# dselivanov/rsparse

Hardware: AMD Instinct MI355X
Metric: als_iterations_per_sec (higher is better)
Workload: dtype f32 (Gram products of rows > 512 / <= 32 non-zeros as 2 x fp16 / 3 x bf16 split terms of the fp32 operands, fp32 accumulate; everything else fp32); 1 GPU; WRMF implicit ALS, CG(3), synthetic 10000000x1000000, 500155883 nnz, rank 128, lambda 0.1; survey_config=3, feedback=implicit, n_items=1000000, nnz=500155883, rank=128, solver=conjugate_gradient, cg_steps=3, parallelism=rows sharded x1, factors replicated

## Files before the change

rsparse_amd/csrc/wrmf_cgp.hip:

```cpp
#include "wrmf_internal.h"
#include "wrmf_device.h"

namespace rsparse_hip {
namespace {

using namespace dev;

constexpr int kPairMaxSweeps = 4;

template <int NQ, bool QUAD = false>
struct PairSmem {
  static constexpr int KP = 128, ps = KP + 8, os = QUAD ? KP + 8 : KP + 4;
  static constexpr int cols = QUAD ? 16 : 8;
  static constexpr int pcs = QUAD ? 2 * ps : ps;
  static constexpr size_t gfrag = NQ == 16 ? (size_t)4 * 16 * 1024 : 0;
  static constexpr size_t nxt = NQ == 16 ? (size_t)4 * 2 * 2 * 64 * 4 : 0;
  static constexpr size_t pub = (size_t)2 * cols * ps * 2, out = (size_t)cols * os * 4;
  static_assert(!QUAD || (pub == out && (size_t)pcs * 2 == (size_t)os * 4), "QUAD: one column, one stretch of LDS");
  static constexpr size_t bytes = gfrag + (QUAD ? pub : pub + out) + (size_t)4 * 8 * NQ * 4 + nxt + 16;
};
static_assert(PairSmem<16>::bytes <= 81920 && PairSmem<16, true>::bytes <= 81920, "two workgroups per CU");

template <bool GB, bool KFULL = false, int NQ = 8, bool QUAD = false>
__global__ __launch_bounds__(256, 2) void als_cgp_kernel(AlsArgs a, const int32_t* __restrict__ rows, int n_rows, int iters,
// ... 294 lines not shown
            } else {
              ah = *reinterpret_cast<const f16x8*>(sGf + ((t * 4 + ks) * 2 + 0) * 1024 + (QUAD ? ln : lane) * 16);
              al = *reinterpret_cast<const f16x8*>(sGf + ((t * 4 + ks) * 2 + 1) * 1024 + (QUAD ? ln : lane) * 16);
            }
            d0[t] = __builtin_amdgcn_mfma_f32_16x16x32_f16(ah, bh, d0[t], 0, 0, 0);
            d1[t] = __builtin_amdgcn_mfma_f32_16x16x32_f16(ah, bl, d1[t], 0, 0, 0);
            d1[t] = __builtin_amdgcn_mfma_f32_16x16x32_f16(al, bh, d1[t], 0, 0, 0);
          }
        }
        if (QUAD || (lane & 15) < 8) {
#pragma unroll
          for (int t = 0; t < 2; t++) {
            const f32x4 d = (d0[t] + d1[t]) * ginv;
            float* po = QUAD ? sOut + li * SM::os + 32 * wv + 16 * t + 4 * lg : sOut + (lane & 15) * SM::os + 32 * wv + 16 * t + 4 * (lane >> 4);
            *reinterpret_cast<f32x4*>(po) = d;
          }
        }
      }
      float lacc = 0.f;
      if (mode != 2) {
        float* trec = (mode == 0 ? tacc : tcur) + gs;
#pragma unroll
        for (int q0 = 0; q0 < NQ; q0 += 4) {
          if (blk_on(q0)) {
            float t[4];
            f32x2 s2[4];
#pragma unroll
            for (int u = 0; u < 4; u++) s2[u] = f32x2{0.f, 0.f};
#pragma unroll
            for (int rr = 0; rr < RPN; rr += 2) {
              const f32x2 va = {v[rr], v[rr + 1]};
#pragma unroll
              for (int u = 0; u < 4; u++) {
                const f32x2 xa = {xt[q0 + u][rr], xt[q0 + u][rr + 1]};
                s2[u] = __builtin_elementwise_fma(xa, va, s2[u]);
              }
            }
#pragma unroll
            for (int u = 0; u < 4; u++) t[u] = s2[u].x + s2[u].y;
#pragma unroll
            for (int u = 0; u < 4; u++) t[u] += dpp<0xB1>(t[u]);
#pragma unroll
            for (int u = 0; u < 4; u++) t[u] += dpp<0x4E>(t[u]);
#pragma unroll
            for (int u = 0; u < 4; u++) t[u] += dpp<0x141>(t[u]);
#pragma unroll
            for (int u = 0; u < 4; u++) t[u] += dpp<0x140>(t[u]);
#pragma unroll
            for (int u = 0; u < 4; u++) {
              const int q = q0 + u;
              const float c = GREG ? cv[q] : (QUAD ? nx[64 + q] : nx[64 + 2 * q + g2]);
              trec[SS * q] = t[u];
              const float w = mode == 0 ? c - (c - 1.f) * (GB ? t[u] + gbias : t[u]) : (c - 1.f) * t[u];
#pragma unroll
              for (int rr = 0; rr < RPN; rr++) acc[rr] = fmaf(w, xt[q][rr], acc[rr]);
            }
          }
        }
      } else {
        wave_sync();
        const float t = tacc[lslot];
        const float dd = ltgt - t;
        const float ls = row16_sum((lgrp && lslot < cnt) ? cl * dd * dd : 0.f);
        lacc = QUAD ? ls : pair_sum(ls);
      }
      if (mode != 2) {
        __syncthreads();
        const float f = (QUAD || g2 == 0) ? vinv : 0.f;
#pragma unroll
        for (int b = 0; b < NV; b++) {
          const float* po = QUAD ? sOut + lcol * SM::os + b * 16 * VW + li * VW : sOut + col * SM::os + b * 16 * VW + i * VW;
          const f32x4 o = *reinterpret_cast<const f32x4*>(po);
#pragma unroll
          for (int c = 0; c < VW; c++) acc[b * VW + c] = fmaf(f, o[c], acc[b * VW + c]);
        }
#pragma unroll
        for (int rr = 0; rr < RPN; rr++) out[rr] = QUAD ? acc[rr] : pair_sum(acc[rr]);
        if constexpr (GB) {
          if (mode == 0) {
#pragma unroll
            for (int b = 0; b < NV; b++) {
              const int off = b * 16 * VW + i * VW;
              const float4 pc = *reinterpret_cast<const float4*>(a.rhs_init + min(off, k - VW));
              const float* pf = reinterpret_cast<const float*>(&pc);
#pragma unroll
              for (int c = 0; c < VW; c++) out[b * VW + c] += off < k ? pf[c] : 0.f;
            }
          }
        }
      } else {
        loss_out = lacc;
      }
    };
    auto dot16 = [&](const float(&u)[RPN], const float(&w)[RPN]) {
      float s = 0.f;
#pragma unroll
      for (int rr = 0; rr < RPN; rr++) s = fmaf(u[rr], w[rr], s);
      return row16_sum(s);
    };

    float dummy = 0.f;
    sweep(x, 0, r, dummy);
    if constexpr (KFULL)
      request_indices(it + 1 < iters && ridx(it + 1) < n_rows, p1_c, p2_c - p1_c, (it + 1) & 1);
#pragma unroll
    for (int rr = 0; rr < RPN; rr++) p[rr] = r[rr];
    float rsold = dot16(r, r);
    bool conv = !live;
    for (int itc = 0; itc < a.cg_steps; ++itc) {
      sweep(p, 1, ap, dummy);
      const float pap = dot16(p, ap);
      const float alpha = conv ? 0.f : (float)((double)rsold / (double)pap);
      wave_sync();
      if (lgrp) tacc[lslot] = fmaf(alpha, tcur[lslot], tacc[lslot]);
      wave_sync();
#pragma unroll
      for (int rr = 0; rr < RPN; rr++) {
        x[rr] = fmaf(alpha, p[rr], x[rr]);
        r[rr] = fmaf(-alpha, ap[rr], r[rr]);
      }
      const float rsnew = dot16(r, r);
      if (!conv) {
        if (rsnew < kCgTol) {
          conv = true;
        } else {
          const float beta = (float)((double)rsnew / (double)rsold);
#pragma unroll
          for (int rr = 0; rr < RPN; rr++) p[rr] = fmaf(p[rr], beta, r[rr]);
          rsold = rsnew;
        }
      }
    }
    float rl = 0.f;
    sweep(x, 2, ap, rl);
    if constexpr (KFULL) {
      settle_indices();
    }
    if (live) {
      const float xx = dot16(x, x);
      wloss += (double)rl + a.lambda_loss * (double)xx;
      if (QUAD || g2 == 0) {
#pragma unroll
        for (int b = 0; b < NV; b++) {
          const int off = b * 16 * VW + i * VW;
          if (off < k) {
            float4 pc;
            float* pf = reinterpret_cast<float*>(&pc);
#pragma unroll
            for (int c = 0; c < VW; c++) pf[c] = x[b * VW + c];
            *reinterpret_cast<float4*>(yrow + off) = pc;
          }
        }
      }
    }
  }
  const double other = __shfl(wloss, 32);
  if constexpr (QUAD) {
    const double wsum = (wloss + __shfl(wloss, 16)) + (other + __shfl(wloss, 48));
    if (lane == 0) a.loss_partials[loss_slot0 + (size_t)blockIdx.x * 4 + wv] = wsum;
  } else {
    if (lane == 0) a.loss_partials[loss_slot0 + (size_t)blockIdx.x * 4 + wv] = wloss + other;
  }
}

}

bool cgp_supported(int k, bool implicit) { return implicit && k > 64 && k <= 128 && k % 4 == 0; }
bool cgp_wide_supported(int k, bool implicit, bool gbias) { return implicit && k == 128 && !gbias; }
bool cgp_quad_supported(int k, bool implicit, bool gbias) { return implicit && k == 128 && !gbias; }

hipError_t launch_als_cgp(const AlsArgs& a, const int32_t* rows, int n_rows, CgpForm form, size_t loss_slot0, hipStream_t s,
                          hipEvent_t* ev_slot) {
  const int rpw = cgp_rows_per_wave(form);
  const int grid = cgp_grid(n_rows, rpw);
  if (grid <= 0) return hipSuccess;
  const int iters = cgp_visits(n_rows, rpw);
  const bool gb = a.gbias != 0.f;
  const bool full = !gb && a.k == 128;
  const bool wide = form == kCgpWide, quad = form == kCgpQuad;
  if ((wide || quad) && !full) return hipErrorInvalidValue;
  auto k0 = als_cgp_kernel<false, false>;
  auto k0f = als_cgp_kernel<false, true>;
  auto k1 = als_cgp_kernel<true, false>;
  auto kw = als_cgp_kernel<false, true, 16>;
  auto kq = als_cgp_kernel<false, true, 16, true>;
  const void* fn = quad ? reinterpret_cast<const void*>(kq) : wide ? reinterpret_cast<const void*>(kw)
                        : gb ? reinterpret_cast<const void*>(k1) : (full ? reinterpret_cast<const void*>(k0f) : reinterpret_cast<const void*>(k0));
  const size_t lds = quad ? PairSmem<16, true>::bytes : wide ? PairSmem<16>::bytes : PairSmem<8>::bytes;
  hipError_t err = hipFuncSetAttribute(fn, hipFuncAttributeMaxDynamicSharedMemorySize, (int)lds);
  if (err != hipSuccess) return err;
  prof_note(ev_slot, fn);
  if (quad) hipLaunchKernelGGL(kq, dim3(grid), dim3(256), lds, s, a, rows, n_rows, iters, loss_slot0);
  else if (wide) hipLaunchKernelGGL(kw, dim3(grid), dim3(256), lds, s, a, rows, n_rows, iters, loss_slot0);
  else if (gb) hipLaunchKernelGGL(k1, dim3(grid), dim3(256), lds, s, a, rows, n_rows, iters, loss_slot0);
  else if (full) hipLaunchKernelGGL(k0f, dim3(grid), dim3(256), lds, s, a, rows, n_rows, iters, loss_slot0);
  else hipLaunchKernelGGL(k0, dim3(grid), dim3(256), lds, s, a, rows, n_rows, iters, loss_slot0);
  return hipGetLastError();
}

}
```

rsparse_amd/csrc/wrmf_cgq.hip:

```cpp
#include <algorithm>

#include "wrmf_internal.h"
#include "wrmf_device.h"

namespace rsparse_hip {
namespace {

using namespace dev;

constexpr int kGvFirstMinCapq = 16;
constexpr int kStreamPrefixQ = 4;
constexpr int kIdxPrefetchMaxWpr = 2;

constexpr int kMaxSavedSweeps = 4;

template <int KP>
struct QG {
  static constexpr int RPN = KP / 16;
  static constexpr int VW = RPN >= 4 ? 4 : RPN;
  static constexpr int NV = RPN / VW;
  __device__ static __forceinline__ int elem(int i, int r) { return (r / VW) * (16 * VW) + i * VW + (r % VW); }
};

template <int VW>
struct Piece;
template <>
struct Piece<4> { using type = float4; };
template <>
struct Piece<2> { using type = float2; };

__device__ __forceinline__ float groups_reduce_scatter4(const float a0, const float a1, const float a2, const float a3) {
  const auto s01 = __builtin_amdgcn_permlane16_swap(__float_as_uint(a0), __float_as_uint(a1), false, false);
  const float c = __uint_as_float(s01[0]) + __uint_as_float(s01[1]);
  const auto s23 = __builtin_amdgcn_permlane16_swap(__float_as_uint(a2), __float_as_uint(a3), false, false);
  const float d = __uint_as_float(s23[0]) + __uint_as_float(s23[1]);
  const auto t = __builtin_amdgcn_permlane32_swap(__float_as_uint(c), __float_as_uint(d), false, false);
  return __uint_as_float(t[0]) + __uint_as_float(t[1]);
}
template <int KP, int CAPQ, int WAVES, int WPR, int STREAM, bool IMPLICIT, int DMF = 0>
struct QSmem {
  static constexpr size_t gram_floats = (IMPLICIT && DMF != 1) ? (size_t)KP * KP : 0;
  static constexpr size_t vec_floats = IMPLICIT ? (size_t)WAVES * KP : 0;
  static constexpr size_t red_floats = WPR > 1 ? (size_t)2 * WAVES * KP + 2 * WAVES : 0;
  static constexpr bool cv_lds = !STREAM && CAPQ * (KP / 16) > 128;
  static constexpr bool wideq = !STREAM && CAPQ * (KP / 16) > 160;
  static constexpr size_t tsv_floats = (STREAM && !IMPLICIT) ? 0 : (size_t)WAVES * (cv_lds ? 3 : 2) * CAPQ * 4;
  static constexpr size_t pre_floats = STREAM ? (size_t)WAVES * kStreamPrefixQ * 4 * KP : 0;
  static constexpr int dmf_ps = KP + 8, dmf_os = KP + 4;
  static constexpr size_t dmf_floats = DMF ? (size_t)WAVES * dmf_ps + (size_t)WAVES * dmf_os : 0;
  static constexpr size_t pfx_floats =
      (!STREAM && WPR > kIdxPrefetchMaxWpr && (CAPQ == 16 || CAPQ == 20 || CAPQ == 24)) ? (size_t)WAVES * 2 * CAPQ * 4 : 0;
  static constexpr size_t wl_floats = cv_lds ? (size_t)WAVES * 2 : 0;
  static constexpr size_t xs_floats = cv_lds ? (size_t)WAVES * KP : 0;
  static constexpr size_t bytes =
      (gram_floats + vec_floats + red_floats + tsv_floats + pre_floats + dmf_floats + pfx_floats + wl_floats + xs_floats) * 4 + 16;
};

template <int KP, int CAPQ, int WAVES, int WPR, int STREAM, bool IMPLICIT, int DMF = 0, bool GB = false, bool KFULL = false>
__global__ __launch_bounds__(WAVES * 64, 2) void als_cgq_kernel(AlsArgs a, const int32_t* __restrict__ rows, int n_rows,
                                                             int rows_per_team, size_t loss_slot0) {
  using G_ = QG<KP>;
  constexpr int RPN = G_::RPN, VW = G_::VW, NV = G_::NV, CAP = CAPQ * 4, TEAMS = WAVES / WPR;
  using piece_t = typename Piece<VW>::type;
  using SM = QSmem<KP, CAPQ, WAVES, WPR, STREAM, IMPLICIT, DMF>;
  static_assert(WAVES % WPR == 0, "teams must tile the workgroup");
  constexpr bool GRS = RPN == 8 && VW == 4;
  auto groups_all_reduce8 = [](float(&a8)[RPN]) {
    if constexpr (RPN == 8) {
      const float r0 = groups_reduce_scatter4(a8[0], a8[1], a8[2], a8[3]);
      const float r1 = groups_reduce_scatter4(a8[4], a8[5], a8[6], a8[7]);
      float g0[4], g1[4];
      rows_to_all<4>(r0, g0);
      rows_to_all<4>(r1, g1);
#pragma unroll
      for (int e = 0; e < 4; e++) a8[e] = g0[e], a8[4 + e] = g1[e];
    }
  };
  static_assert(!DMF || (IMPLICIT && KP == 128 && WAVES == 4 && WPR == 1 && STREAM == 0), "DMF geometry");
  static_assert(DMF != 1 || CAPQ == 8, "register-resident G terms: only the 8-quad kernel has the 64 registers");
  static_assert(!GB || IMPLICIT, "the global bias of explicit feedback is removed from the data (R/model_WRMF.R:278-282)");
  const float gbias = GB ? a.gbias : 0.f, ltgt = GB ? a.loss_tgt_const : 1.f;
  extern __shared__ __attribute__((aligned(16))) char smem[];
  float* sG = reinterpret_cast<float*>(smem);
  float* sVec = sG + SM::gram_floats;
  float* sRed = sVec + SM::vec_floats;
  float* sRedL = sRed + (WPR > 1 ? 2 * WAVES * KP : 0);
  float* sTsv = sVec + SM::vec_floats + SM::red_floats;
  float* sPre = sTsv + SM::tsv_floats;
  float* sPfx = sPre + SM::pre_floats;
  _Float16* sPh = reinterpret_cast<_Float16*>(sPre + SM::pre_floats);
  _Float16* sPl = sPh + WAVES * SM::dmf_ps;
  float* sOut = reinterpret_cast<float*>(sPl + WAVES * SM::dmf_ps);

  const int tid = threadIdx.x, lane = tid & 63, wv = rfl(tid >> 6);
  const int g = lane >> 4, i = lane & 15;
  const int team = wv / WPR, tw = wv % WPR;
  const int k = KFULL ? KP : a.k;
  if constexpr (IMPLICIT && DMF == 0) {
    constexpr int GU = (KP * KP) % (8 * WAVES * 64) == 0 ? 8 : ((KP * KP) % (2 * WAVES * 64) == 0 ? 2 : 1);
    static_assert((KP * KP) % (GU * WAVES * 64) == 0, "the Gramian copy walks whole batches");
    for (int e0 = tid; e0 < KP * KP; e0 += GU * WAVES * 64) {
      float gv[GU];
#pragma unroll
      for (int u = 0; u < GU; u++) {
        const int e = e0 + u * WAVES * 64, r = e / KP, c = e % KP;
        gv[u] = a.XtX[(size_t)min(r, k - 1) * k + min(c, k - 1)];
      }
#pragma unroll
      for (int u = 0; u < GU; u++) {
// ... 138 lines not shown
    float cl[CVLDS ? 1 : NSL];
#pragma unroll
    for (int s2 = 0; s2 < (CVLDS ? 1 : NSL); s2++) cl[s2] = 0.f;
    auto csv_fill = [&](auto&& conf_of, const int n) {
      const int ln = opaque_lane<WIDEQ>(lane);
#pragma unroll
      for (int s2 = 0; s2 < NSL; s2++) {
        const int sl = ln + 64 * s2;
        if (s2 == 0 || sl < CAP) csv[(sl & 3) * CAPQ + (sl >> 2)] = sl < n ? conf_of(sl) : 0.f;
      }
    };
    int ccnt = 0;

    constexpr bool ZPAD = STREAM == 0;
    constexpr bool TSAVE = STREAM == 0;
    constexpr bool GVFIRST = STREAM == 0 && CAPQ >= kGvFirstMinCapq;
    constexpr bool IDXPF = CAP <= 64 && ((STREAM == 0 && WPR <= kIdxPrefetchMaxWpr) || (STREAM == 1 && IMPLICIT));
    constexpr bool DMAPF = KFULL && !IDXPF && SM::pfx_floats > 0;
    int* pfxI = reinterpret_cast<int*>(sPfx) + wv * 2 * CAP;
    float* pfxC = sPfx + wv * 2 * CAP + CAP;
    auto dma_slot = [&](const int j0, const int n) {
      const int j = j0 + min(lane, n - 1);
      dma4(a.row_idx + j, lds_addr(pfxI));
      dma4(a.vals + j, lds_addr(pfxC));
      if constexpr (CAP > 64) {
        if (lane < CAP - 64) {
          const int j2 = j0 + min(lane + 64, n - 1);
          dma4(a.row_idx + j2, lds_addr(pfxI + 64));
          dma4(a.vals + j2, lds_addr(pfxC + 64));
        }
      }
    };
    int pf_pos = -1;
#define RSP_SLOT_IN(q, n) (SM::wideq ? g < (n) - 4 * (q) : 4 * (q) + g < (n))
#define RSP_SLOT_J(q, n) max(SM::wideq ? min(g, (n) - 1 - 4 * (q)) + 4 * (q) : min(4 * (q) + g, (n) - 1), 0)
    auto gather_q = [&](auto nq_tag, const int base, const int n, const bool from_pf = false) {
      constexpr int NQG = decltype(nq_tag)::value;
      int id[NQG > 0 ? NQG : 1];
      if constexpr (DMAPF) {
        if (!from_pf && n > 0) {
          dma_slot(base, n);
          wait_vm<0>();
        }
        wave_sync();
#pragma unroll
        for (int q = 0; q < NQG; q++) {
          const int j = RSP_SLOT_J(q, n);
          id[q] = pfxI[j];
          if constexpr (!CVLDS) cv[q] = (!ZPAD || RSP_SLOT_IN(q, n)) ? pfxC[j] : 0.f;
        }
        if constexpr (CVLDS) {
          csv_fill([&](int sl) { return pfxC[sl]; }, n);
        } else if constexpr (TSAVE) {
#pragma unroll
          for (int s2 = 0; s2 < NSL; s2++) cl[s2] = lane + 64 * s2 < n ? pfxC[min(lane + 64 * s2, CAP - 1)] : 0.f;
        }
        wave_sync();
      } else if (IDXPF && from_pf) {
        int* xi = reinterpret_cast<int*>(tacc);
        wave_sync();
        xi[lane & (CAP - 1)] = pf_id;
        tcur[lane & (CAP - 1)] = pf_c;
        wave_sync();
#pragma unroll
        for (int q = 0; q < NQG; q++) {
          const int j = RSP_SLOT_J(q, n);
          id[q] = xi[j];
          if constexpr (!CVLDS) cv[q] = (!ZPAD || RSP_SLOT_IN(q, n)) ? tcur[j] : 0.f;
        }
        if constexpr (TSAVE) cl[0] = lane < n ? pf_c : 0.f;
        wave_sync();
      } else {
#pragma unroll
        for (int q = 0; q < NQG; q++) {
          const int j = RSP_SLOT_J(q, n);
          id[q] = a.row_idx[base + j];
          if constexpr (!CVLDS) {
            const float c = a.vals[base + j];
            cv[q] = (!ZPAD || RSP_SLOT_IN(q, n)) ? c : 0.f;
          }
        }
        if constexpr (CVLDS) {
          wave_sync();
          csv_fill([&](int sl) { return a.vals[base + sl]; }, n);
          wave_sync();
        } else if constexpr (TSAVE) {
#pragma unroll
          for (int s2 = 0; s2 < NSL; s2++) cl[s2] = lane + 64 * s2 < n ? a.vals[base + lane + 64 * s2] : 0.f;
        }
      }
      const int ig = (SM::wideq && !KFULL) ? (opaque_lane<true>(lane) & 15) : i;
#pragma unroll
      for (int q = 0; q < NQG; q++) {
        const float* src = (!ZPAD || RSP_SLOT_IN(q, n)) ? a.X + (size_t)id[q] * k : a.zero_row;
#pragma unroll
        for (int b = 0; b < NV; b++) {
          const int off = b * 16 * VW + ig * VW;
          if constexpr (KFULL) {
            const piece_t pc = *reinterpret_cast<const piece_t*>(src + off);
            const float* pf = reinterpret_cast<const float*>(&pc);
#pragma unroll
            for (int c = 0; c < VW; c++) xt[q][b * VW + c] = pf[c];
          } else {
            const piece_t pc = *reinterpret_cast<const piece_t*>(src + min(off, k - VW));
            const float* pf = reinterpret_cast<const float*>(&pc);
#pragma unroll
            for (int c = 0; c < VW; c++) xt[q][b * VW + c] = off < k ? pf[c] : 0.f;
          }
// ... 66 lines not shown

    if constexpr (!WS_FIRST) load_warm_start();

    auto quad_pass = [&](const float(&v)[RPN], const int mode, float(&acc)[RPN], float& lacc, float* tsave) {
      float* trec = (mode == 0 ? tacc : tcur) + g;
      constexpr int QB = 4;
#pragma unroll
      for (int q0 = 0; q0 < CAPQ; q0 += QB) {
        if (4 * q0 < ccnt) {
          float t[QB];
          f32x2 s2[QB];
#pragma unroll
          for (int u = 0; u < QB; u++) s2[u] = f32x2{0.f, 0.f};
#pragma unroll
          for (int rr = 0; rr < RPN; rr += 2) {
            const f32x2 va = {v[rr], v[rr + 1]};
#pragma unroll
            for (int u = 0; u < QB; u++) {
              const f32x2 xa = {xt[q0 + u][rr], xt[q0 + u][rr + 1]};
              s2[u] = __builtin_elementwise_fma(xa, va, s2[u]);
            }
          }
#pragma unroll
          for (int u = 0; u < QB; u++) t[u] = s2[u].x + s2[u].y;
#pragma unroll
          for (int u = 0; u < QB; u++) t[u] += dpp<0xB1>(t[u]);
#pragma unroll
          for (int u = 0; u < QB; u++) t[u] += dpp<0x4E>(t[u]);
#pragma unroll
          for (int u = 0; u < QB; u++) t[u] += dpp<0x141>(t[u]);
#pragma unroll
          for (int u = 0; u < QB; u++) t[u] += dpp<0x140>(t[u]);
          float cq[QB];
          if constexpr (CVLDS) {
            const float4 c4 = *reinterpret_cast<const float4*>(csv + g * CAPQ + q0);
            cq[0] = c4.x; cq[1] = c4.y; cq[2] = c4.z; cq[3] = c4.w;
          } else {
#pragma unroll
            for (int u = 0; u < QB; u++) cq[u] = cv[q0 + u];
          }
#pragma unroll
          for (int u = 0; u < QB; u++) {
            const int q = q0 + u;
            const bool valid = ZPAD || 4 * q + g < ccnt;
            const float c = cq[u];
            if constexpr (STREAM == 1) {
              if (tsave && valid && i == 0) tsave[4 * q + g] = t[u];
            } else if constexpr (TSAVE) {
              trec[4 * q] = t[u];
            }
            if (mode == 2) {
              const float d = IMPLICIT ? ltgt - t[u] : c - t[u];
              lacc += valid ? (IMPLICIT ? c * d * d : d * d) : 0.f;
            } else {
              float w;
              if (mode == 0) w = IMPLICIT ? c - (c - 1.f) * (GB ? t[u] + gbias : t[u]) : c - t[u];
              else w = IMPLICIT ? (c - 1.f) * t[u] : t[u];
              w = valid ? w : 0.f;
#pragma unroll
              for (int rr = 0; rr < RPN; rr++) acc[rr] = fmaf(w, xt[q][rr], acc[rr]);
            }
          }
        }
      }
    };

    auto sweep = [&](const float(&v)[RPN], const int mode, float(&out)[RPN], float& loss_out, const bool live,
                     const int sidx = 0) {
      float acc[RPN];
#pragma unroll
      for (int rr = 0; rr < RPN; rr++) acc[rr] = 0.f;
      float lacc = 0.f;
      float vinv = 0.f;
      if constexpr (DMF) {
        if (mode != 2) {
          float vmax = 0.f;
#pragma unroll
          for (int rr = 0; rr < RPN; rr++) vmax = fmaxf(vmax, fabsf(v[rr]));
          vmax = row16_max(vmax);
          const int ve = fp16_scale_exp(vmax);
          const float vs = __uint_as_float((unsigned)ve << 23);
          vinv = __uint_as_float((unsigned)(254 - ve) << 23) * (mode == 0 ? -1.f : 1.f);
          if (g < NV) {
            float w4[VW];
#pragma unroll
            for (int c = 0; c < VW; c++) w4[c] = (g == 0 ? v[c] : v[VW + c]) * vs;
            unsigned h0, l0, h1, l1;
            split_f16(w4[0], w4[1], h0, l0);
            split_f16(w4[2], w4[3], h1, l1);
            const int off = wv * SM::dmf_ps + g * 16 * VW + i * VW;
            *reinterpret_cast<uint2*>(sPh + off) = make_uint2(h0, h1);
            *reinterpret_cast<uint2*>(sPl + off) = make_uint2(l0, l1);
          }
          __syncthreads();
          f32x4 d0[2], d1[2];
#pragma unroll
          for (int t = 0; t < 2; t++) d0[t] = d1[t] = f32x4{0.f, 0.f, 0.f, 0.f};
          const int nb = (lane & 3) * SM::dmf_ps + 8 * (lane >> 4);
#pragma unroll
          for (int ks = 0; ks < 4; ks++) {
            const f16x8 bh = *reinterpret_cast<const f16x8*>(sPh + nb + 32 * ks);
            const f16x8 bl = *reinterpret_cast<const f16x8*>(sPl + nb + 32 * ks);
#pragma unroll
            for (int t = 0; t < 2; t++) {
              f16x8 ah, al;
              if constexpr (DMF == 1) {
                ah = gAh[t][ks];
                al = gAl[t][ks];
              } else {
                ah = *reinterpret_cast<const f16x8*>(sGf + ((t * 4 + ks) * 2 + 0) * 1024 + lane * 16);
                al = *reinterpret_cast<const f16x8*>(sGf + ((t * 4 + ks) * 2 + 1) * 1024 + lane * 16);
              }
              d0[t] = __builtin_amdgcn_mfma_f32_16x16x32_f16(ah, bh, d0[t], 0, 0, 0);
              d1[t] = __builtin_amdgcn_mfma_f32_16x16x32_f16(ah, bl, d1[t], 0, 0, 0);
              d1[t] = __builtin_amdgcn_mfma_f32_16x16x32_f16(al, bh, d1[t], 0, 0, 0);
            }
          }
          if ((lane & 15) < 4) {
#pragma unroll
            for (int t = 0; t < 2; t++) {
              const f32x4 d = (d0[t] + d1[t]) * ginv;
              *reinterpret_cast<f32x4*>(sOut + (lane & 15) * SM::dmf_os + 32 * wv + 16 * t + 4 * (lane >> 4)) = d;
            }
          }
        }
      }
      if (live) {
        if constexpr (IMPLICIT && !DMF) {
          if (mode != 2) {
            wave_sync();
            if (g == 0) {
#pragma unroll
              for (int b = 0; b < NV; b++) {
                piece_t pc;
                float* pf = reinterpret_cast<float*>(&pc);
#pragma unroll
                for (int c = 0; c < VW; c++) pf[c] = v[b * VW + c];
                *reinterpret_cast<piece_t*>(vec + b * 16 * VW + i * VW) = pc;
              }
            }
            wave_sync();
          }
        }
        auto dense_part = [&]() {
          if (IMPLICIT && !DMF && mode != 2) {
            const float sign = mode == 0 ? -1.f : 1.f;
            if constexpr (NRES > 0) {
#pragma unroll
              for (int rs = 0; rs < NRES; rs++) {
                const int kk = 4 * (g + 4 * rs);
                const float4 vb = *reinterpret_cast<const float4*>(vec + kk);
                const float vv[4] = {sign * vb.x, sign * vb.y, sign * vb.z, sign * vb.w};
#pragma unroll
                for (int u = 0; u < 4; u++)
#pragma unroll
                  for (int b = 0; b < NV; b++) {
                    const float* pf = reinterpret_cast<const float*>(&gres[rs][u][b]);
#pragma unroll
                    for (int c = 0; c < VW; c++) acc[b * VW + c] = fmaf(vv[u], pf[c], acc[b * VW + c]);
                  }
              }
            }
            for (int s4 = tw * 4 + g + 4 * NRES; s4 < KP / 4; s4 += WPR * 4) {
              const int kk = 4 * s4;
              const float4 vb = *reinterpret_cast<const float4*>(vec + kk);
              const float vv[4] = {sign * vb.x, sign * vb.y, sign * vb.z, sign * vb.w};
#pragma unroll
              for (int u = 0; u < 4; u++) {
                const float* grow = sG + (kk + u) * KP;
#pragma unroll
                for (int b = 0; b < NV; b++) {
                  const piece_t pc = *reinterpret_cast<const piece_t*>(grow + b * 16 * VW + i * VW);
                  const float* pf = reinterpret_cast<const float*>(&pc);
#pragma unroll
                  for (int c = 0; c < VW; c++) acc[b * VW + c] = fmaf(vv[u], pf[c], acc[b * VW + c]);
                }
              }
            }
          }
        };
        if constexpr (GVFIRST) dense_part();
        if (resident) {
          if (mode != 2 || !TSAVE) {
            quad_pass(v, mode, acc, lacc, nullptr);
          } else {
            wave_sync();
            float esum = 0.f;
            const int ln = opaque_lane<WIDEQ>(lane);
#pragma unroll
            for (int s2 = 0; s2 < NSL; s2++) {
              const int sl = NSL == 1 ? (lane & (CAP - 1)) : min(ln + 64 * s2, CAP - 1);
              const float t = tacc[sl];
              const float clv = CVLDS ? csv[(sl & 3) * CAPQ + (sl >> 2)] : cl[s2];
              const float d = IMPLICIT ? ltgt - t : clv - t;
              const float e = IMPLICIT ? clv * d * d : d * d;
              esum += ln + 64 * s2 < ccnt ? e : 0.f;
            }
            lacc = row16_sum(esum);
          }
        } else if (mode == 2 && tscr) {
          for (int ch = tw; ch < (cnt + CAP - 1) / CAP; ch += WPR) {
            const int n = min(CAP, cnt - ch * CAP);
            if (lane < n) {
              const size_t pos = (size_t)ch * CAP + lane;
              float t = tscr[pos];
#pragma unroll
              for (int s2 = 0; s2 < kMaxSavedSweeps; s2++)
                if (s2 < a.cg_steps && alph[s2] != 0.f) t = fmaf(alph[s2], tscr[(size_t)(s2 + 1) * a.stream_nnz + pos], t);
              const float c = a.vals[p1 + pos];
              const float d = IMPLICIT ? ltgt - t : c - t;
              lacc += IMPLICIT ? c * d * d : d * d;
            }
          }
          lacc = row16_sum(lacc);
        } else {
          if (pw > 0) {
            prefix_chunk(mode == 0);
            ccnt = pw;
            quad_pass(v, mode, acc, lacc, tscr ? tscr + (size_t)sidx * a.stream_nnz + (size_t)tw * PCAP : nullptr);
          }
          for (int ch = tw; ch < nchunks; ch += WPR) {
            ccnt = min(CAP, cnt - pre - ch * CAP);
            gather(p1 + pre + ch * CAP, ccnt, IDXPF && pf_pos == ch && pf_cnt == ccnt);
            if constexpr (IDXPF) {
              const int nch = ch + WPR < nchunks ? ch + WPR : tw;
              const int ncc = min(CAP, cnt - pre - nch * CAP);
              const int j = p1 + pre + nch * CAP + min(lane & (CAP - 1), ncc - 1);
              pf_id = a.row_idx[j];
              pf_c = a.vals[j];
              pf_cnt = ncc;
              pf_pos = nch;
            }
            quad_pass(v, mode, acc, lacc,
                      tscr ? tscr + (size_t)sidx * a.stream_nnz + (size_t)pre + (size_t)ch * CAP : nullptr);
          }
        }
        if constexpr (!GVFIRST) dense_part();
        if constexpr (!DMF) {
          if (mode != 2) {
            if constexpr (GRS) {
              if constexpr (WPR == 1) groups_all_reduce8(acc);
            } else {
#pragma unroll
              for (int rr = 0; rr < RPN; rr++) acc[rr] = groups_sum(acc[rr]);
            }
          } else {
            lacc = groups_sum(lacc);
          }
        }
      }
      if constexpr (DMF) {
        if (mode != 2) {
          __syncthreads();
          const float f = g == 0 ? vinv : 0.f;
#pragma unroll
          for (int b = 0; b < NV; b++) {
            const f32x4 o = *reinterpret_cast<const f32x4*>(sOut + wv * SM::dmf_os + b * 16 * VW + i * VW);
#pragma unroll
            for (int c = 0; c < VW; c++) acc[b * VW + c] = fmaf(f, o[c], acc[b * VW + c]);
          }
          if constexpr (GRS) {
            groups_all_reduce8(acc);
          } else {
#pragma unroll
            for (int rr = 0; rr < RPN; rr++) acc[rr] = groups_sum(acc[rr]);
          }
        } else {
          lacc = groups_sum(lacc);
        }
      }
      if constexpr (WPR > 1) {
        float* red = sRed + buf * WAVES * KP;
        if (mode != 2) {
          if constexpr (GRS) {
            const float r0 = groups_reduce_scatter4(acc[0], acc[1], acc[2], acc[3]);
            const float r1 = groups_reduce_scatter4(acc[4], acc[5], acc[6], acc[7]);
            red[wv * KP + 4 * i + g] = r0;
            red[wv * KP + 64 + 4 * i + g] = r1;
          } else if (g == 0) {
#pragma unroll
            for (int b = 0; b < NV; b++) {
              piece_t pc;
              float* pf = reinterpret_cast<float*>(&pc);
#pragma unroll
              for (int c = 0; c < VW; c++) pf[c] = acc[b * VW + c];
              *reinterpret_cast<piece_t*>(red + wv * KP + b * 16 * VW + i * VW) = pc;
            }
          }
        } else if (lane == 0) {
          sRedL[buf * WAVES + wv] = lacc;
        }
        __syncthreads();
        if (mode != 2) {
#pragma unroll
          for (int rr = 0; rr < RPN; rr++) acc[rr] = 0.f;
#pragma unroll
          for (int w2 = 0; w2 < WPR; w2++) {
#pragma unroll
            for (int b = 0; b < NV; b++) {
              const piece_t pc = *reinterpret_cast<const piece_t*>(red + (team * WPR + w2) * KP + b * 16 * VW + i * VW);
              const float* pf = reinterpret_cast<const float*>(&pc);
#pragma unroll
              for (int c = 0; c < VW; c++) acc[b * VW + c] += pf[c];
            }
          }
        } else {
          lacc = 0.f;
#pragma unroll
          for (int w2 = 0; w2 < WPR; w2++) lacc += sRedL[buf * WAVES + team * WPR + w2];
        }
        buf ^= 1;
      } else {
        __builtin_amdgcn_sched_barrier(0);
      }
      if (mode != 2) {
#pragma unroll
        for (int rr = 0; rr < RPN; rr++) out[rr] = acc[rr];
        if constexpr (GB) {
          if (mode == 0) {
#pragma unroll
            for (int b = 0; b < NV; b++) {
              const int off = b * 16 * VW + i * VW;
              const piece_t pc = *reinterpret_cast<const piece_t*>(a.rhs_init + min(off, k - VW));
              const float* pf = reinterpret_cast<const float*>(&pc);
#pragma unroll
              for (int c = 0; c < VW; c++) out[b * VW + c] += off < k ? pf[c] : 0.f;
            }
          }
        }
        if constexpr (!IMPLICIT) {
#pragma unroll
          for (int rr = 0; rr < RPN; rr++) out[rr] = fmaf(mode == 0 ? -lam_use : lam_use, v[rr], out[rr]);
        }
      } else {
        loss_out = lacc;
      }
    };

    auto dot16 = [&](const float(&u)[RPN], const float(&w)[RPN]) {
      float s = 0.f;
#pragma unroll
      for (int rr = 0; rr < RPN; rr++) s = fmaf(u[rr], w[rr], s);
      return row16_sum(s);
    };

    const bool live = have && (GB || cnt > 0);
    float dummy = 0.f;
    sweep(x, 0, r, dummy, live);
    auto x_piece = [&](const int b) { return reinterpret_cast<piece_t*>(xs + b * 16 * VW + i * VW); };
    if constexpr (CVLDS) {
      if (g == 0) {
#pragma unroll
        for (int b = 0; b < NV; b++) {
          piece_t pc;
          float* pf = reinterpret_cast<float*>(&pc);
#pragma unroll
          for (int c = 0; c < VW; c++) pf[c] = x[b * VW + c];
          *x_piece(b) = pc;
        }
      }
    }
    if constexpr (META_LATE) RSP_ADVANCE_META()
#undef RSP_ADVANCE_META
    if constexpr (IDXPF && STREAM == 0) {
      if (it + 1 < rows_per_team && row_index(it + 1) < n_rows) {
        const int np1 = rfl(p1_c), ncnt = rfl(p2_c) - np1;
        const int nper = min(CAP, (((ncnt + WPR - 1) / WPR) + 15) & ~15);
        const int ncc = max(0, min(nper, ncnt - tw * nper));
        if (ncc > 0) {
          const int j = np1 + tw * nper + min(lane & (CAP - 1), ncc - 1);
          pf_id = a.row_idx[j];
          pf_c = a.vals[j];
          pf_cnt = ncc;
        }
      }
    }
    if constexpr (DMAPF) {
      if (it + 1 < rows_per_team && row_index(it + 1) < n_rows) {
        const int np1 = rfl(p1_c), ncnt = rfl(p2_c) - np1;
        const int nper = min(CAP, (((ncnt + WPR - 1) / WPR) + 15) & ~15);
        const int ncc = max(0, min(nper, ncnt - tw * nper));
        if (ncc > 0) {
          dma_slot(np1 + tw * nper, ncc);
          pf_cnt = ncc;
        }
      }
    }
#pragma unroll
    for (int rr = 0; rr < RPN; rr++) p[rr] = r[rr];
    float rsold = dot16(r, r);
    bool conv = false;
    for (int itc = 0; itc < a.cg_steps; ++itc) {
      if (WPR == 1 && !DMF && conv) break;
      sweep(p, 1, ap, dummy, live && !conv, itc + 1);
      if (!conv) {
        const float pap = dot16(p, ap);
        const float alpha = (float)((double)rsold / (double)pap);
#pragma unroll
        for (int s2 = 0; s2 < kMaxSavedSweeps; s2++)
          if (s2 == itc) alph[s2] = alpha;
        if constexpr (TSAVE) {
          wave_sync();
          const int ln = opaque_lane<WIDEQ>(lane);
#pragma unroll
          for (int s2 = 0; s2 < NSL; s2++) {
            const int sl = NSL == 1 ? (lane & (CAP - 1)) : ln + 64 * s2;
            if (CAP % 64 == 0 || sl < CAP) tacc[sl] = fmaf(alpha, tcur[sl], tacc[sl]);
          }
          wave_sync();
        }
        if constexpr (CVLDS) {
          if (g == 0) {
#pragma unroll
            for (int b = 0; b < NV; b++) {
              piece_t pc = *x_piece(b);
              float* pf = reinterpret_cast<float*>(&pc);
#pragma unroll
              for (int c = 0; c < VW; c++) pf[c] = fmaf(alpha, p[b * VW + c], pf[c]);
              *x_piece(b) = pc;
            }
          }
        }
#pragma unroll
        for (int rr = 0; rr < RPN; rr++) {
          if constexpr (!CVLDS) x[rr] = fmaf(alpha, p[rr], x[rr]);
          r[rr] = fmaf(-alpha, ap[rr], r[rr]);
        }
        const float rsnew = dot16(r, r);
        if (rsnew < kCgTol) {
          conv = true;
        } else {
          const float beta = (float)((double)rsnew / (double)rsold);
#pragma unroll
          for (int rr = 0; rr < RPN; rr++) p[rr] = fmaf(p[rr], beta, r[rr]);
          rsold = rsnew;
        }
      }
    }
    if constexpr (CVLDS) {
      wave_sync();
#pragma unroll
      for (int b = 0; b < NV; b++) {
        const piece_t pc = *x_piece(b);
        const float* pf = reinterpret_cast<const float*>(&pc);
#pragma unroll
        for (int c = 0; c < VW; c++) x[b * VW + c] = pf[c];
      }
    }
    float rl = 0.f;
    sweep(x, 2, ap, rl, live);
    if constexpr (META_LATE) p1_c = rfl(p1_c), p2_c = rfl(p2_c);
    if constexpr (DMAPF) wait_vm<0>();
    if constexpr (IDXPF && STREAM == 0) {
      asm volatile("" : "+v"(pf_id), "+v"(pf_c));
    }
    if (live && tw == 0) {
      const float xx = dot16(x, x);
      const double wl_row = IMPLICIT ? (double)rl + a.lambda_loss * (double)xx : (double)(rl + lam_use * xx);
      if constexpr (CVLDS) {
        if (lane == 0) *wl_lds += wl_row;
      } else {
        wloss += wl_row;
      }
      if (g == 0) {
#pragma unroll
        for (int b = 0; b < NV; b++) {
          const int off = b * 16 * VW + i * VW;
          if (off < k) {
            piece_t pc;
            float* pf = reinterpret_cast<float*>(&pc);
#pragma unroll
            for (int c = 0; c < VW; c++) pf[c] = x[b * VW + c];
            *reinterpret_cast<piece_t*>(yrow + off) = pc;
          }
        }
      }
    }
  }
  if (lane == 0) a.loss_partials[loss_slot0 + (size_t)blockIdx.x * WAVES + wv] = CVLDS ? *wl_lds : wloss;
}

struct BucketDef { int waves, wpr, capq, stream, max_len; };
constexpr int kNB = 6;
constexpr int kNCfg = 2;
constexpr BucketDef kBuckets[kNCfg][kNB] = {
    {{8, 8, 16, 1, 0x7fffffff}, {8, 8, 16, 0, 512}, {4, 4, 16, 0, 256}, {4, 2, 16, 0, 128}, {4, 1, 16, 0, 64}, {4, 1, 8, 0, 32}},
    {{8, 8, 16, 1, 0x7fffffff}, {4, 4, 32, 0, 512}, {4, 2, 32, 0, 256}, {4, 1, 32, 0, 128}, {4, 1, 16, 0, 64}, {4, 1, 8, 0, 32}},
};
constexpr int cfg_of_kp(int KP) { return KP == 64 ? 1 : 0; }
constexpr int kTeam4Waves = 4, kTeam4Capq = 20;
static_assert(kTeam4Max == kTeam4Waves * kTeam4Capq * 4, "wrmf_internal.h's split and the kernel's capacity");
// ... 258 lines not shown
```

Before: 8.529 iterations/s.

## Compute only p·Ap scalar in final CG step instead of full matrix-vector product

In the last conjugate-gradient step only alpha is needed, so a new sweep mode 3 accumulates the scalar p·A·p directly (sum of w*t plus the dense Gram term dotted with p) rather than building the full Ap vector. This skips the per-row vector accumulation, reductions across waves and the residual and beta updates in the final step. A per-configuration table chooses whether this reduced step runs inside or after the loop, or whether the full step is kept. Several lane-index expressions are also routed through opaque_lane to steer codegen.

```diff
diff --git a/rsparse_amd/csrc/wrmf_cgp.hip b/rsparse_amd/csrc/wrmf_cgp.hip
--- a/rsparse_amd/csrc/wrmf_cgp.hip
+++ b/rsparse_amd/csrc/wrmf_cgp.hip
@@ -370,6 +370,10 @@
               const float c = GREG ? cv[q] : (QUAD ? nx[64 + q] : nx[64 + 2 * q + g2]);
               trec[SS * q] = t[u];
               const float w = mode == 0 ? c - (c - 1.f) * (GB ? t[u] + gbias : t[u]) : (c - 1.f) * t[u];
+              if (mode == 3) {
+                lacc = fmaf(w, t[u], lacc);
+                continue;
+              }
 #pragma unroll
               for (int rr = 0; rr < RPN; rr++) acc[rr] = fmaf(w, xt[q][rr], acc[rr]);
             }
@@ -385,6 +389,19 @@
       if (mode != 2) {
         __syncthreads();
         const float f = (QUAD || g2 == 0) ? vinv : 0.f;
+        if (mode == 3) {
+          float dl = 0.f;
+#pragma unroll
+          for (int b = 0; b < NV; b++) {
+            const float* po = QUAD ? sOut + lcol * SM::os + b * 16 * VW + li * VW : sOut + col * SM::os + b * 16 * VW + i * VW;
+            const f32x4 o = *reinterpret_cast<const f32x4*>(po);
+#pragma unroll
+            for (int c = 0; c < VW; c++) dl = fmaf(o[c], v[b * VW + c], dl);
+          }
+          lacc = fmaf(f, row16_sum(dl), lacc);
+          loss_out = QUAD ? lacc : pair_sum(lacc);
+          return;
+        }
 #pragma unroll
         for (int b = 0; b < NV; b++) {
           const float* po = QUAD ? sOut + lcol * SM::os + b * 16 * VW + li * VW : sOut + col * SM::os + b * 16 * VW + i * VW;
@@ -425,7 +442,7 @@
     for (int rr = 0; rr < RPN; rr++) p[rr] = r[rr];
     float rsold = dot16(r, r);
     bool conv = !live;
-    for (int itc = 0; itc < a.cg_steps; ++itc) {
+    for (int itc = 0; itc + 1 < a.cg_steps; ++itc) {
       sweep(p, 1, ap, dummy);
       const float pap = dot16(p, ap);
       const float alpha = conv ? 0.f : (float)((double)rsold / (double)pap);
@@ -449,6 +466,16 @@
         }
       }
     }
+    if (a.cg_steps > 0) {
+      float pap = 0.f;
+      sweep(p, 3, ap, pap);
+      const float alpha = conv ? 0.f : (float)((double)rsold / (double)pap);
+      wave_sync();
+      if (lgrp) tacc[lslot] = fmaf(alpha, tcur[lslot], tacc[lslot]);
+      wave_sync();
+#pragma unroll
+      for (int rr = 0; rr < RPN; rr++) x[rr] = fmaf(alpha, p[rr], x[rr]);
+    }
     float rl = 0.f;
     sweep(x, 2, ap, rl);
     if constexpr (KFULL) {
@@ -473,11 +500,12 @@
     }
   }
   const double other = __shfl(wloss, 32);
+  const bool first_lane = __lane_id() == 0;
   if constexpr (QUAD) {
     const double wsum = (wloss + __shfl(wloss, 16)) + (other + __shfl(wloss, 48));
-    if (lane == 0) a.loss_partials[loss_slot0 + (size_t)blockIdx.x * 4 + wv] = wsum;
+    if (first_lane) a.loss_partials[loss_slot0 + (size_t)blockIdx.x * 4 + wv] = wsum;
   } else {
-    if (lane == 0) a.loss_partials[loss_slot0 + (size_t)blockIdx.x * 4 + wv] = wloss + other;
+    if (first_lane) a.loss_partials[loss_slot0 + (size_t)blockIdx.x * 4 + wv] = wloss + other;
   }
 }
 
diff --git a/rsparse_amd/csrc/wrmf_cgq.hip b/rsparse_amd/csrc/wrmf_cgq.hip
--- a/rsparse_amd/csrc/wrmf_cgq.hip
+++ b/rsparse_amd/csrc/wrmf_cgq.hip
@@ -55,6 +55,41 @@
   static constexpr size_t bytes =
       (gram_floats + vec_floats + red_floats + tsv_floats + pre_floats + dmf_floats + pfx_floats + wl_floats + xs_floats) * 4 + 16;
 };
+
+constexpr int kLastFull = 0, kLastDotsInLoop = 1, kLastDotsBehind = 2;
+struct LastStepChoice { int kp, capq, waves, wpr, stream; bool implicit; int dmf; bool gb, kfull; int form; };
+constexpr LastStepChoice kLastStepChoices[] = {
+    {64, 32, 4, 1, 0, true, 0, true, false, kLastFull},
+    {64, 16, 4, 1, 0, true, 0, true, true, kLastFull},
+    {64, 32, 4, 1, 0, true, 0, false, true, kLastFull},
+    {64, 16, 4, 1, 0, true, 0, false, false, kLastFull},
+    {64, 16, 4, 1, 0, false, 0, false, true, kLastFull},
+    {128, 16, 8, 8, 0, true, 0, true, true, kLastFull},
+    {128, 16, 8, 8, 0, true, 0, true, false, kLastFull},
+    {128, 16, 4, 2, 0, true, 0, true, true, kLastFull},
+    {128, 16, 4, 1, 0, true, 2, true, true, kLastFull},
+    {128, 16, 8, 8, 0, true, 0, false, false, kLastFull},
+    {32, 8, 4, 1, 0, false, 0, false, true, kLastDotsBehind},
+    {64, 32, 4, 2, 0, true, 0, true, false, kLastDotsBehind},
+    {64, 32, 4, 2, 0, true, 0, false, false, kLastDotsBehind},
+    {128, 16, 4, 4, 0, true, 0, true, false, kLastDotsBehind},
+    {128, 16, 4, 2, 0, true, 0, true, false, kLastDotsBehind},
+    {128, 24, 4, 4, 0, true, 0, false, true, kLastDotsBehind},
+    {128, 24, 4, 4, 0, true, 0, false, false, kLastDotsBehind},
+    {128, 20, 4, 4, 0, true, 0, false, true, kLastDotsBehind},
+    {128, 20, 4, 4, 0, true, 0, false, false, kLastDotsBehind},
+    {128, 16, 4, 4, 0, true, 0, false, false, kLastDotsBehind},
+    {128, 16, 4, 2, 0, true, 0, false, false, kLastDotsBehind},
+    {128, 16, 4, 1, 0, true, 2, false, false, kLastDotsBehind},
+    {128, 20, 4, 4, 0, false, 0, false, true, kLastDotsBehind},
+};
+constexpr int last_step_form(int KP, int CAPQ, int WAVES, int WPR, int STREAM, bool IMPLICIT, int DMF, bool GB, bool KFULL) {
+  for (const LastStepChoice& c : kLastStepChoices)
+    if (c.kp == KP && c.capq == CAPQ && c.waves == WAVES && c.wpr == WPR && c.stream == STREAM && c.implicit == IMPLICIT &&
+        c.dmf == DMF && c.gb == GB && c.kfull == KFULL)
+      return c.form;
+  return kLastDotsInLoop;
+}
 
 template <int KP, int CAPQ, int WAVES, int WPR, int STREAM, bool IMPLICIT, int DMF = 0, bool GB = false, bool KFULL = false>
 __global__ __launch_bounds__(WAVES * 64, 2) void als_cgq_kernel(AlsArgs a, const int32_t* __restrict__ rows, int n_rows,
@@ -299,8 +334,9 @@
         if constexpr (CVLDS) {
           csv_fill([&](int sl) { return pfxC[sl]; }, n);
         } else if constexpr (TSAVE) {
-#pragma unroll
-          for (int s2 = 0; s2 < NSL; s2++) cl[s2] = lane + 64 * s2 < n ? pfxC[min(lane + 64 * s2, CAP - 1)] : 0.f;
+          const int lo = opaque_lane<true>(lane);
+#pragma unroll
+          for (int s2 = 0; s2 < NSL; s2++) cl[s2] = lane + 64 * s2 < n ? pfxC[min(lo + 64 * s2, CAP - 1)] : 0.f;
         }
         wave_sync();
       } else if (IDXPF && from_pf) {
@@ -473,6 +509,9 @@
             if (mode == 2) {
               const float d = IMPLICIT ? ltgt - t[u] : c - t[u];
               lacc += valid ? (IMPLICIT ? c * d * d : d * d) : 0.f;
+            } else if (mode == 3) {
+              const float w = IMPLICIT ? (c - 1.f) * t[u] : t[u];
+              lacc = fmaf(valid ? w : 0.f, t[u], lacc);
             } else {
               float w;
               if (mode == 0) w = IMPLICIT ? c - (c - 1.f) * (GB ? t[u] + gbias : t[u]) : c - t[u];
@@ -492,6 +531,7 @@
 #pragma unroll
       for (int rr = 0; rr < RPN; rr++) acc[rr] = 0.f;
       float lacc = 0.f;
+      float dl = 0.f;
       float vinv = 0.f;
       if constexpr (DMF) {
         if (mode != 2) {
@@ -517,7 +557,8 @@
           f32x4 d0[2], d1[2];
 #pragma unroll
           for (int t = 0; t < 2; t++) d0[t] = d1[t] = f32x4{0.f, 0.f, 0.f, 0.f};
-          const int nb = (lane & 3) * SM::dmf_ps + 8 * (lane >> 4);
+          const int ln = opaque_lane<DMF == 2>(lane);
+          const int nb = (ln & 3) * SM::dmf_ps + 8 * (ln >> 4);
 #pragma unroll
           for (int ks = 0; ks < 4; ks++) {
             const f16x8 bh = *reinterpret_cast<const f16x8*>(sPh + nb + 32 * ks);
@@ -529,19 +570,19 @@
                 ah = gAh[t][ks];
                 al = gAl[t][ks];
               } else {
-                ah = *reinterpret_cast<const f16x8*>(sGf + ((t * 4 + ks) * 2 + 0) * 1024 + lane * 16);
-                al = *reinterpret_cast<const f16x8*>(sGf + ((t * 4 + ks) * 2 + 1) * 1024 + lane * 16);
+                ah = *reinterpret_cast<const f16x8*>(sGf + ((t * 4 + ks) * 2 + 0) * 1024 + ln * 16);
+                al = *reinterpret_cast<const f16x8*>(sGf + ((t * 4 + ks) * 2 + 1) * 1024 + ln * 16);
               }
               d0[t] = __builtin_amdgcn_mfma_f32_16x16x32_f16(ah, bh, d0[t], 0, 0, 0);
               d1[t] = __builtin_amdgcn_mfma_f32_16x16x32_f16(ah, bl, d1[t], 0, 0, 0);
               d1[t] = __builtin_amdgcn_mfma_f32_16x16x32_f16(al, bh, d1[t], 0, 0, 0);
             }
           }
-          if ((lane & 15) < 4) {
+          if ((ln & 15) < 4) {
 #pragma unroll
             for (int t = 0; t < 2; t++) {
               const f32x4 d = (d0[t] + d1[t]) * ginv;
-              *reinterpret_cast<f32x4*>(sOut + (lane & 15) * SM::dmf_os + 32 * wv + 16 * t + 4 * (lane >> 4)) = d;
+              *reinterpret_cast<f32x4*>(sOut + (ln & 15) * SM::dmf_os + 32 * wv + 16 * t + 4 * (ln >> 4)) = d;
             }
           }
         }
@@ -600,7 +641,13 @@
             }
           }
         };
-        if constexpr (GVFIRST) dense_part();
+        if constexpr (GVFIRST) {
+          dense_part();
+          if (mode == 3) {
+#pragma unroll
+            for (int rr = 0; rr < RPN; rr++) dl = fmaf(acc[rr], v[rr], dl);
+          }
+        }
         if (resident) {
           if (mode != 2 || !TSAVE) {
             quad_pass(v, mode, acc, lacc, nullptr);
@@ -656,9 +703,18 @@
                       tscr ? tscr + (size_t)sidx * a.stream_nnz + (size_t)pre + (size_t)ch * CAP : nullptr);
           }
         }
-        if constexpr (!GVFIRST) dense_part();
+        if constexpr (!GVFIRST) {
+          dense_part();
+          if (mode == 3) {
+#pragma unroll
+            for (int rr = 0; rr < RPN; rr++) dl = fmaf(acc[rr], v[rr], dl);
+          }
+        }
         if constexpr (!DMF) {
-          if (mode != 2) {
+          if (mode == 3) {
+            if constexpr (IMPLICIT) lacc += row16_sum(dl);
+            lacc = groups_sum(lacc);
+          } else if (mode != 2) {
             if constexpr (GRS) {
               if constexpr (WPR == 1) groups_all_reduce8(acc);
             } else {
@@ -678,9 +734,14 @@
           for (int b = 0; b < NV; b++) {
             const f32x4 o = *reinterpret_cast<const f32x4*>(sOut + wv * SM::dmf_os + b * 16 * VW + i * VW);
 #pragma unroll
-            for (int c = 0; c < VW; c++) acc[b * VW + c] = fmaf(f, o[c], acc[b * VW + c]);
-          }
-          if constexpr (GRS) {
+            for (int c = 0; c < VW; c++) {
+              if (mode == 3) dl = fmaf(o[c], v[b * VW + c], dl);
+              else acc[b * VW + c] = fmaf(f, o[c], acc[b * VW + c]);
+            }
+          }
+          if (mode == 3) {
+            lacc = groups_sum(fmaf(f, row16_sum(dl), lacc));
+          } else if constexpr (GRS) {
             groups_all_reduce8(acc);
           } else {
 #pragma unroll
@@ -692,7 +753,7 @@
       }
       if constexpr (WPR > 1) {
         float* red = sRed + buf * WAVES * KP;
-        if (mode != 2) {
+        if (mode < 2) {
           if constexpr (GRS) {
             const float r0 = groups_reduce_scatter4(acc[0], acc[1], acc[2], acc[3]);
             const float r1 = groups_reduce_scatter4(acc[4], acc[5], acc[6], acc[7]);
@@ -712,7 +773,7 @@
           sRedL[buf * WAVES + wv] = lacc;
         }
         __syncthreads();
-        if (mode != 2) {
+        if (mode < 2) {
 #pragma unroll
           for (int rr = 0; rr < RPN; rr++) acc[rr] = 0.f;
 #pragma unroll
@@ -734,7 +795,7 @@
       } else {
         __builtin_amdgcn_sched_barrier(0);
       }
-      if (mode != 2) {
+      if (mode < 2) {
 #pragma unroll
         for (int rr = 0; rr < RPN; rr++) out[rr] = acc[rr];
         if constexpr (GB) {
@@ -754,6 +815,14 @@
           for (int rr = 0; rr < RPN; rr++) out[rr] = fmaf(mode == 0 ? -lam_use : lam_use, v[rr], out[rr]);
         }
       } else {
+        if constexpr (!IMPLICIT) {
+          if (mode == 3) {
+            float vv = 0.f;
+#pragma unroll
+            for (int rr = 0; rr < RPN; rr++) vv = fmaf(v[rr], v[rr], vv);
+            lacc = fmaf(lam_use, row16_sum(vv), lacc);
+          }
+        }
         loss_out = lacc;
       }
     };
@@ -811,42 +880,55 @@
     for (int rr = 0; rr < RPN; rr++) p[rr] = r[rr];
     float rsold = dot16(r, r);
     bool conv = false;
+#define RSP_STEP_X(alpha, step)                                                                   \
+    do {                                                                                          \
+      _Pragma("unroll") for (int s2 = 0; s2 < kMaxSavedSweeps; s2++)                              \
+        if (s2 == (step)) alph[s2] = (alpha);                                                     \
+      if constexpr (TSAVE) {                                                                      \
+        wave_sync();                                                                              \
+        const int ln = opaque_lane<WIDEQ>(lane);                                                  \
+        _Pragma("unroll") for (int s2 = 0; s2 < NSL; s2++) {                                      \
+          const int sl = NSL == 1 ? (lane & (CAP - 1)) : ln + 64 * s2;                            \
+          if (CAP % 64 == 0 || sl < CAP) tacc[sl] = fmaf((alpha), tcur[sl], tacc[sl]);            \
+        }                                                                                         \
+        wave_sync();                                                                              \
+      }                                                                                           \
+      if constexpr (CVLDS) {                                                                      \
+        if (g == 0) {                                                                             \
+          _Pragma("unroll") for (int b = 0; b < NV; b++) {                                        \
+            piece_t pc = *x_piece(b);                                                             \
+            float* pf = reinterpret_cast<float*>(&pc);                                            \
+            _Pragma("unroll") for (int c = 0; c < VW; c++) pf[c] = fmaf((alpha), p[b * VW + c], pf[c]); \
+            *x_piece(b) = pc;                                                                     \
+          }                                                                                       \
+        }                                                                                         \
+      } else {                                                                                    \
+        _Pragma("unroll") for (int rr = 0; rr < RPN; rr++) x[rr] = fmaf((alpha), p[rr], x[rr]);   \
+      }                                                                                           \
+    } while (0)
+#define RSP_LAST_STEP()                                                                           \
+    do {                                                                                          \
+      float pap = 0.f;                                                                            \
+      sweep(p, 3, ap, pap, live && !conv, a.cg_steps);                                            \
+      if (!conv) {                                                                                \
+        const float alpha = (float)((double)rsold / (double)pap);                                 \
+        RSP_STEP_X(alpha, a.cg_steps - 1);                                                        \
+      }                                                                                           \
+    } while (0)
+    constexpr int LAST = last_step_form(KP, CAPQ, WAVES, WPR, STREAM, IMPLICIT, DMF, GB, KFULL);
     for (int itc = 0; itc < a.cg_steps; ++itc) {
       if (WPR == 1 && !DMF && conv) break;
+      if (LAST != kLastFull && itc + 1 == a.cg_steps) {
+        if constexpr (LAST == kLastDotsInLoop) RSP_LAST_STEP();
+        break;
+      }
       sweep(p, 1, ap, dummy, live && !conv, itc + 1);
       if (!conv) {
         const float pap = dot16(p, ap);
         const float alpha = (float)((double)rsold / (double)pap);
-#pragma unroll
-        for (int s2 = 0; s2 < kMaxSavedSweeps; s2++)
-          if (s2 == itc) alph[s2] = alpha;
-        if constexpr (TSAVE) {
-          wave_sync();
-          const int ln = opaque_lane<WIDEQ>(lane);
-#pragma unroll
-          for (int s2 = 0; s2 < NSL; s2++) {
-            const int sl = NSL == 1 ? (lane & (CAP - 1)) : ln + 64 * s2;
-            if (CAP % 64 == 0 || sl < CAP) tacc[sl] = fmaf(alpha, tcur[sl], tacc[sl]);
-          }
-          wave_sync();
-        }
-        if constexpr (CVLDS) {
-          if (g == 0) {
-#pragma unroll
-            for (int b = 0; b < NV; b++) {
-              piece_t pc = *x_piece(b);
-              float* pf = reinterpret_cast<float*>(&pc);
-#pragma unroll
-              for (int c = 0; c < VW; c++) pf[c] = fmaf(alpha, p[b * VW + c], pf[c]);
-              *x_piece(b) = pc;
-            }
-          }
-        }
-#pragma unroll
-        for (int rr = 0; rr < RPN; rr++) {
-          if constexpr (!CVLDS) x[rr] = fmaf(alpha, p[rr], x[rr]);
-          r[rr] = fmaf(-alpha, ap[rr], r[rr]);
-        }
+        RSP_STEP_X(alpha, itc);
+#pragma unroll
+        for (int rr = 0; rr < RPN; rr++) r[rr] = fmaf(-alpha, ap[rr], r[rr]);
         const float rsnew = dot16(r, r);
         if (rsnew < kCgTol) {
           conv = true;
@@ -858,6 +940,11 @@
         }
       }
     }
+    if constexpr (LAST == kLastDotsBehind) {
+      if (a.cg_steps > 0 && !(WPR == 1 && !DMF && conv)) RSP_LAST_STEP();
+    }
+#undef RSP_LAST_STEP
+#undef RSP_STEP_X
     if constexpr (CVLDS) {
       wave_sync();
 #pragma unroll
```

Result: faster. 8.715 iterations/s, median of 6 (+2.2%).
